# nikhilTkur/Multigrid_Nikhil_C-

Measured on AMD Instinct MI355X. Metric: fine_grid_stencil_updates_per_sec, higher is better.
Workload: dtype f64

## Files before the change

### multigrid_nikhil_c-_amd/csrc/mgx.hip

```cpp

#include "../../include/mgx.h"
#include "mgx_bottom.hpp"
#include "mgx_kernels.hpp"
#include "mgx_launch.hpp"
#include "mgx_var.hpp"
#include "mgx_galerkin.hpp"
#include "mgx_opdep.hpp"
#include "mgx_cheby.hpp"
#include "mgx_line.hpp"
#include "mgx_small.hpp"
#include "mgx_krylov.hpp"
#include "mgx_dist_plan.hpp"

#include <chrono>
#include <unistd.h>
#include <cmath>
#include <cstdio>
#include <cstdlib>
#include <cstring>
#include <string>
#include <vector>

namespace {

// ... 2018 lines not shown
    hipStream_t st = (hipStream_t)stream;
    int flips = 0;
    const int nb = with_kernel_set(q.f64, smoother, f->arith, [&](auto k) {
        using K = decltype(k);
        using T = typename K::T;
        return fold_block<T, K::SM, K::AR>(fc, q, (T*)u, (const T*)b, (T*)tmp, pitch, omega, c, (const T*)coarse_e,
                                           (T*)coarse_b, nullptr, crow_lo, crow_hi, restrict_mode, scratch, st, &flips);
    });
    if (nb < 0) return MGX_ERR_INVALID;
    if (post == 2) hipLaunchKernelGGL(k_reduce_partials, dim3(1), dim3(kReduceThreads), 0, st, scratch, nb, sum_dev);
    if (result_in_tmp) *result_in_tmp = flips & 1;
    return hipGetLastError() == hipSuccess ? MGX_OK : MGX_ERR_HIP;
}

int mgx_slab_restrict(const mgx_slab* f, const void* u, const void* b, const mgx_slab* c, void* cb, void* zero_u,
                      int crow_lo, int crow_hi, int restrict_mode, int fused, void* stream)
{
    if (slab_check(f) || slab_check(c) || !b || !cb || (fused && !u)) return MGX_ERR_INVALID;
    if (restrict_mode != MGX_RESTRICT_CONSISTENT && restrict_mode != MGX_RESTRICT_FW16) return MGX_ERR_INVALID;
    if (c->level != f->level - 1 || c->dtype != f->dtype) return MGX_ERR_INVALID;
    const int N = 1 << f->level;
    const long pitch = level_pitch(f->level, f->dtype), cpitch = level_pitch(c->level, c->dtype);
    const int off = 2 * c->row0 - f->row0;
    const int halo = fused ? 2 : 1;
    if (crow_lo < 0 || crow_hi > c->rows || crow_lo + c->row0 < 1 || crow_hi + c->row0 > N / 2) return MGX_ERR_INVALID;
    if (crow_hi > crow_lo && (2 * crow_lo + off - halo < 0 || 2 * (crow_hi - 1) + off + halo > f->rows - 1)) return MGX_ERR_INVALID;
    const int rpc = env_int("MGX_ROWS", 0);
    if (f->dtype == MGX_DTYPE_F64)
        launch_restrict<double>((const double*)u, (const double*)b, (double*)cb, (double*)zero_u, N, pitch, cpitch,
                                crow_lo, crow_hi, off, restrict_mode, fused != 0, rpc, (hipStream_t)stream);
    else
        launch_restrict<float>((const float*)u, (const float*)b, (float*)cb, (float*)zero_u, N, pitch, cpitch,
                               crow_lo, crow_hi, off, restrict_mode, fused != 0, rpc, (hipStream_t)stream);
    return hipGetLastError() == hipSuccess ? MGX_OK : MGX_ERR_HIP;
}

int mgx_slab_prolong(const mgx_slab* f, void* u, const mgx_slab* c, const void* e, int row_lo, int row_hi, int add,
                     void* stream)
{
    if (slab_check(f) || slab_check(c) || !u || !e) return MGX_ERR_INVALID;
    if (c->level != f->level - 1 || c->dtype != f->dtype) return MGX_ERR_INVALID;
    const int N = 1 << f->level;
    const long pitch = level_pitch(f->level, f->dtype), cpitch = level_pitch(c->level, c->dtype);
    const int off = 2 * c->row0 - f->row0;
    if (row_lo < 0 || row_hi > f->rows || row_lo + f->row0 < 1 || row_hi + f->row0 > N) return MGX_ERR_INVALID;
    if (row_hi > row_lo) {
        const int ylo = row_lo - off, yhi = row_hi - 1 - off;
        if (ylo < 0 || (yhi >> 1) + (yhi & 1) > c->rows - 1) return MGX_ERR_INVALID;
    }
    const int rpc = env_int("MGX_ROWS", 0);
    if (f->dtype == MGX_DTYPE_F64)
        launch_prolong<double>((double*)u, (const double*)e, N, pitch, cpitch, row_lo, row_hi, off, add != 0, rpc, (hipStream_t)stream);
    else
        launch_prolong<float>((float*)u, (const float*)e, N, pitch, cpitch, row_lo, row_hi, off, add != 0, rpc, (hipStream_t)stream);
    return hipGetLastError() == hipSuccess ? MGX_OK : MGX_ERR_HIP;
}

int mgx_slab_residual_sumsq(const mgx_slab* s, const void* u, const void* b, int row_lo, int row_hi,
                            double* scratch, double* sum_dev, void* stream)
{
    if (slab_check(s) || !u || !b || !scratch || !sum_dev) return MGX_ERR_INVALID;
    const int N = 1 << s->level;
    const long pitch = level_pitch(s->level, s->dtype);
    if (row_lo < 1 || row_hi > s->rows - 1 || row_lo + s->row0 < 1 || row_hi + s->row0 > N || row_hi <= row_lo) return MGX_ERR_INVALID;
    const int rpc = env_int("MGX_ROWS", 0);
    if (s->dtype == MGX_DTYPE_F64)
        launch_residual<double, 1>((const double*)u, (const double*)b, nullptr, 0, scratch, sum_dev, 1.0, N, pitch, row_lo, row_hi, rpc, (hipStream_t)stream, -1, s->rows);
    else
        launch_residual<float, 1>((const float*)u, (const float*)b, nullptr, 0, scratch, sum_dev, 1.0, N, pitch, row_lo, row_hi, rpc, (hipStream_t)stream, -1, s->rows);
    return hipGetLastError() == hipSuccess ? MGX_OK : MGX_ERR_HIP;
}

int mgx_create_rank(const mgx_config* cfg, int rank, int world, const void* rccl_id, const mgx_transport* transport,
                    mgx_handle* out)
{
    if (!cfg || !out) { g_create_error = "null argument"; return MGX_ERR_INVALID; }
    *out = nullptr;
    if (cfg->smoother == MGX_SMOOTHER_CHEBYSHEV) {
        g_create_error = "MGX_SMOOTHER_CHEBYSHEV: single-GPU handles of op = MGX_OPERATOR_STENCIL5 / MGX_OPERATOR_GALERKIN only";
        return MGX_ERR_INVALID;
    }
    if (cfg->smoother >= MGX_SMOOTHER_LINE_X && cfg->smoother <= MGX_SMOOTHER_LINE_ALT) {
        g_create_error = "MGX_SMOOTHER_LINE_X / LINE_Y / LINE_ALT: single-GPU handles of op = MGX_OPERATOR_STENCIL5 / MGX_OPERATOR_GALERKIN only";
        return MGX_ERR_INVALID;
    }
    if (cfg->coarsest_level < 2 || cfg->finest_level < cfg->coarsest_level || cfg->finest_level > 15 ||
        cfg->mu1 < 0 || cfg->mu2 < 0 || !(cfg->omega > 0.0 && cfg->omega < 2.0) || cfg->smoother < 0 || cfg->smoother > 1 ||
        cfg->dtype < 0 || cfg->dtype > 2 || cfg->restrict_mode < 0 || cfg->restrict_mode > 1 || cfg->bottom < 0 || cfg->bottom > 1 || cfg->arith < 0 || cfg->arith > 1 ||
        (rank >= 0 && (world < 1 || rank >= world)) || (rank < 0 && cfg->n_gpus < 2)) {
        g_create_error = "invalid configuration";
        return MGX_ERR_INVALID;
    }
    if (cfg->op != MGX_OPERATOR_POISSON) {
        g_create_error = "multi-GPU handles: op = MGX_OPERATOR_POISSON only (MGX_OPERATOR_STENCIL5 / MGX_OPERATOR_GALERKIN: one GPU)";
        return MGX_ERR_INVALID;
    }
    log_runtime_libs("mgx_create_rank");
    mgx_solver* s = new (std::nothrow) mgx_solver();
    if (!s) { g_create_error = "out of host memory"; return MGX_ERR_ALLOC; }
    s->cfg = *cfg;
    const int rc = dist_create(s, &s->cfg, rank, world, rccl_id, transport);
    if (rc != MGX_OK) { g_create_error = s->err; mgx_destroy(s); return rc; }
    *out = s;
    return MGX_OK;
}

int mgx_runtime_libs(char* buf, size_t cap)
{
    if (!buf || cap == 0) return -1;
    buf[0] = 0;
    FILE* fh = std::fopen("/proc/self/maps", "r");
    if (!fh) return -1;
    std::vector<std::string> seen;
    char line[4096];
    while (std::fgets(line, sizeof line, fh)) {
        const char* path = std::strchr(line, '/');
        if (!path) continue;
        std::string p(path);
        while (!p.empty() && (p.back() == '\n' || p.back() == ' ')) p.pop_back();
        const char* names[] = {"libamdhip64", "libhsa-runtime64", "librccl", "libmgx", "libhiprtc", "libamd_comgr"};
        bool want = false;
        for (const char* n : names) want = want || p.find(n) != std::string::npos;
        if (!want || std::find(seen.begin(), seen.end(), p) != seen.end()) continue;
        seen.push_back(p);
    }
    std::fclose(fh);
    std::string out;
    for (const auto& p : seen) { out += p; out += '\n'; }
    if (out.size() + 1 > cap) out.resize(cap - 1);
    std::memcpy(buf, out.c_str(), out.size() + 1);
    return (int)out.size();
}

int mgx_rccl_unique_id(void* out128)
{
    if (!out128) return MGX_ERR_INVALID;
    ncclUniqueId id;
    if (ncclGetUniqueId(&id) != ncclSuccess) return MGX_ERR_HIP;
    std::memset(out128, 0, 128);
    std::memcpy(out128, &id, sizeof(id) < 128 ? sizeof(id) : 128);
    return MGX_OK;
}

#ifdef MGX_WAVE_TRACE
__attribute__((visibility("default"))) int mgx_debug_wave_trace(void* out, int cap)
{
    int n = 0;
    if (hipDeviceSynchronize() != hipSuccess) return -1;
    if (hipMemcpyFromSymbol(&n, HIP_SYMBOL(mgx::g_wave_trace_n), sizeof(int)) != hipSuccess) return -1;
    n = std::min(std::min(n, cap), 1 << 16);
    if (hipMemcpyFromSymbol(out, HIP_SYMBOL(mgx::g_wave_trace), (size_t)n * sizeof(mgx::WaveTrace)) != hipSuccess) return -1;
    return n;
}
#endif

long mgx_dist_exchanges(mgx_handle s) { return (s && s->dist) ? s->dist->exchanges : -1; }
long mgx_dist_overlapped(mgx_handle s) { return (s && s->dist) ? s->dist->overlapped : -1; }

int mgx_memcpy_d2h(void* dst_host, const void* src_dev, size_t bytes, void* stream)
{
    if (hipMemcpyAsync(dst_host, src_dev, bytes, hipMemcpyDeviceToHost, (hipStream_t)stream) != hipSuccess) return MGX_ERR_HIP;
    return hipStreamSynchronize((hipStream_t)stream) == hipSuccess ? MGX_OK : MGX_ERR_HIP;
}

int mgx_memcpy_h2d(void* dst_dev, const void* src_host, size_t bytes, void* stream)
{
    if (hipMemcpyAsync(dst_dev, src_host, bytes, hipMemcpyHostToDevice, (hipStream_t)stream) != hipSuccess) return MGX_ERR_HIP;
    return hipStreamSynchronize((hipStream_t)stream) == hipSuccess ? MGX_OK : MGX_ERR_HIP;
}

struct mgx_dist_planner { mgx::DistPlanner p; };

int mgx_plan_create(const mgx_config* cfg, int n_slabs, int g, int fold, int deep, mgx_plan_handle* out)
{
    if (!cfg || !out) { g_plan_error = "null argument"; return MGX_ERR_INVALID; }
    *out = nullptr;
    if (cfg->smoother == MGX_SMOOTHER_CHEBYSHEV) {
        g_plan_error = "MGX_SMOOTHER_CHEBYSHEV: the slab plan runs the constant stencil (Jacobi or red-black GS) only";
        return MGX_ERR_INVALID;
    }
    if (cfg->smoother >= MGX_SMOOTHER_LINE_X && cfg->smoother <= MGX_SMOOTHER_LINE_ALT) {
        g_plan_error = "MGX_SMOOTHER_LINE_X / LINE_Y / LINE_ALT: the slab plan runs the constant stencil (Jacobi or red-black GS) only";
        return MGX_ERR_INVALID;
    }
    const int cut = dist_cut_level(*cfg, n_slabs);
    mgx_dist_planner* h = new (std::nothrow) mgx_dist_planner();
    if (!h) return MGX_ERR_ALLOC;
    if (h->p.init(plan_cfg_of(*cfg, n_slabs, g, cut, fold != 0, deep != 0)) != MGX_OK) {
        g_plan_error = h->p.err;
        delete h;
        return MGX_ERR_INVALID;
    }
    *out = h;
    return MGX_OK;
}

int mgx_plan_destroy(mgx_plan_handle p) { delete p; return MGX_OK; }
const char* mgx_plan_last_error(void) { return g_plan_error.c_str(); }
int mgx_plan_cut_level(mgx_plan_handle p) { return p ? p->p.c.cut : -1; }

int mgx_plan_level(mgx_plan_handle p, int level, mgx_dist_level* out)
{
    if (!p || !out || level <= p->p.c.cut || level > p->p.c.finest) return MGX_ERR_INVALID;
    *out = p->p.L(level);
    return MGX_OK;
}

int mgx_plan_cut_share(mgx_plan_handle p, int* row0, int* rows)
{
    if (!p || !row0 || !rows) return MGX_ERR_INVALID;
    *row0 = p->p.c_row0; *rows = p->p.c_rows;
    return MGX_OK;
}

int mgx_plan_guess_set(mgx_plan_handle p, int all_rows)
{
    if (!p) return MGX_ERR_INVALID;
    if (all_rows) p->p.guess_set(); else p->p.guess_changed();
    return MGX_OK;
}

static int plan_emit(mgx_plan_handle p, mgx_dist_op* ops, int cap, bool norm)
{
    if (!p || (!ops && cap > 0)) return MGX_ERR_INVALID;
    std::vector<mgx_dist_op> v;
    mgx::DistPlanner trial = p->p;
    if (norm) trial.emit_norm(v); else trial.emit_vcycle(v);
    if ((int)v.size() > cap) return -(int)v.size();
    p->p = trial;
    for (size_t i = 0; i < v.size(); ++i) ops[i] = v[i];
    return (int)v.size();
}
int mgx_plan_vcycle(mgx_plan_handle p, mgx_dist_op* ops, int cap) { return plan_emit(p, ops, cap, false); }
int mgx_plan_norm(mgx_plan_handle p, mgx_dist_op* ops, int cap) { return plan_emit(p, ops, cap, true); }
int mgx_plan_fmg(mgx_plan_handle p, mgx_dist_op* ops, int cap)
{
    if (!p || (!ops && cap > 0)) return MGX_ERR_INVALID;
    std::vector<mgx_dist_op> v;
    mgx::DistPlanner trial = p->p;
    trial.emit_fmg(v);
    if ((int)v.size() > cap) return -(int)v.size();
    p->p = trial;
    for (size_t i = 0; i < v.size(); ++i) ops[i] = v[i];
    return (int)v.size();
}

}
```

### multigrid_nikhil_c-_amd/csrc/mgx_bottom.hpp

```cpp
#pragma once

#include <hip/hip_runtime.h>
#include <cmath>
#include <vector>

#ifndef MGX_DST_DEEP
#define MGX_DST_DEEP 32
#endif

namespace mgx {

template <typename T, bool FIRST>
__global__ void __launch_bounds__(256)
k_dst_pair(const double* __restrict__ S, const void* __restrict__ Xv, void* __restrict__ Ov, const double* __restrict__ s,
           int n, long gpitch)
{
    __shared__ double prow[256];
    const int j = threadIdx.x;
    const int i = blockIdx.x;
    const bool live = j < n;
    constexpr int kDeep = MGX_DST_DEEP;
    const double* Sr = S + (long)i * n;
    double acc = 0.0;
    {
        int k = 0;
        for (; k + kDeep <= n; k += kDeep) {
            double x[kDeep];
#pragma unroll
            for (int q = 0; q < kDeep; ++q) {
                if constexpr (FIRST) x[q] = live ? (double)(reinterpret_cast<const T*>(Xv)[(long)(k + q + 1) * gpitch + (j + 1)]) : 0.0;
                else x[q] = live ? reinterpret_cast<const double*>(Xv)[(long)(k + q) * n + j] : 0.0;
            }
#pragma unroll
            for (int q = 0; q < kDeep; ++q) acc += Sr[k + q] * x[q];
        }
        double x[kDeep];
#pragma unroll
        for (int q = 0; q < kDeep; ++q) {
            const bool ok = live && (k + q < n);
            if constexpr (FIRST) x[q] = ok ? (double)(reinterpret_cast<const T*>(Xv)[(long)(k + q + 1) * gpitch + (j + 1)]) : 0.0;
            else x[q] = ok ? reinterpret_cast<const double*>(Xv)[(long)(k + q) * n + j] : 0.0;
        }
#pragma unroll
        for (int q = 0; q < kDeep; ++q)
            if (k + q < n) acc += Sr[k + q] * x[q];
    }
    prow[j] = acc;
    __syncthreads();
    double out = 0.0;
    {
        int k = 0;
        for (; k + kDeep <= n; k += kDeep) {
            double x[kDeep];
#pragma unroll
            for (int q = 0; q < kDeep; ++q) x[q] = live ? S[(long)(k + q) * n + j] : 0.0;
#pragma unroll
            for (int q = 0; q < kDeep; ++q) out += prow[k + q] * x[q];
        }
        double x[kDeep];
#pragma unroll
        for (int q = 0; q < kDeep; ++q) x[q] = (live && k + q < n) ? S[(long)(k + q) * n + j] : 0.0;
#pragma unroll
        for (int q = 0; q < kDeep; ++q)
            if (k + q < n) out += prow[k + q] * x[q];
    }
    if (!live) return;
    if constexpr (FIRST) reinterpret_cast<double*>(Ov)[(long)i * n + j] = out / (s[i] + s[j]);
    else reinterpret_cast<T*>(Ov)[(long)(i + 1) * gpitch + (j + 1)] = (T)out;
}

struct BottomDST {
    int n = 0;
    double* S = nullptr;
    double* s = nullptr;
    double* w1 = nullptr;

    hipError_t init(int n_)
    {
        n = n_;
        const size_t nn = (size_t)n * n;
        std::vector<double> hS(nn), hs(n);
        const long double pi = 3.14159265358979323846264338327950288L;
        const long double norm = sqrtl(2.0L / (long double)(n + 1));
        for (int i = 0; i < n; ++i) {
            const long double a = sinl(pi * (long double)(i + 1) / (2.0L * (long double)(n + 1)));
            hs[i] = (double)(4.0L * a * a);
            for (int k = 0; k < n; ++k) {
                const long m = ((long)(i + 1) * (long)(k + 1)) % (2L * (n + 1));
                hS[(size_t)i * n + k] = (double)(norm * sinl(pi * (long double)m / (long double)(n + 1)));
            }
        }
        hipError_t e;
        if ((e = hipMalloc(&S, nn * sizeof(double))) != hipSuccess) return e;
        if ((e = hipMalloc(&s, n * sizeof(double))) != hipSuccess) return e;
        if ((e = hipMalloc(&w1, nn * sizeof(double))) != hipSuccess) return e;
        if ((e = hipMemcpy(S, hS.data(), nn * sizeof(double), hipMemcpyHostToDevice)) != hipSuccess) return e;
        if ((e = hipMemcpy(s, hs.data(), n * sizeof(double), hipMemcpyHostToDevice)) != hipSuccess) return e;
        return hipSuccess;
    }

    void destroy()
    {
        if (S) (void)hipFree(S);
        if (s) (void)hipFree(s);
        if (w1) (void)hipFree(w1);
        S = s = w1 = nullptr;
    }

    template <typename T>
    void solve(const T* b_grid, T* u_grid, long gpitch, hipStream_t st) const
    {
        hipLaunchKernelGGL((k_dst_pair<T, true>), dim3(n), dim3(256), 0, st, S, (const void*)b_grid, (void*)w1, s, n, gpitch);
        hipLaunchKernelGGL((k_dst_pair<T, false>), dim3(n), dim3(256), 0, st, S, (const void*)w1, (void*)u_grid, s, n, gpitch);
    }
};

}
```

### multigrid_nikhil_c-_amd/csrc/mgx_kernels.hpp

```cpp
#pragma once

#include <hip/hip_runtime.h>
#include "mgx_geom.hpp"
#include <stdint.h>
#include <type_traits>

namespace mgx {

template <int B, int E, typename F> __device__ __forceinline__ void static_for(F&& f)
{
    if constexpr (B < E) {
        f(std::integral_constant<int, B>{});
        static_for<B + 1, E>(f);
    }
}

constexpr int kWave = 64;
constexpr int kBlock = 256;
constexpr int kWavesPerBlock = kBlock / kWave;
constexpr int kOutLanes = kWave - 2;

template <typename T> struct VecOf;
template <> struct VecOf<double> { using type = double2; static constexpr int W = 2; };
template <> struct VecOf<float>  { using type = float4;  static constexpr int W = 4; };

__device__ __forceinline__ double2 vzero(double2*) { return make_double2(0.0, 0.0); }
__device__ __forceinline__ float4  vzero(float4*)  { return make_float4(0.f, 0.f, 0.f, 0.f); }

template <typename V> __device__ __forceinline__ V vload(const void* p, bool pred)
{
    V z = vzero((V*)nullptr);
    if (pred) z = *reinterpret_cast<const V*>(p);
    return z;
}
template <typename V> __device__ __forceinline__ void vstore(void* p, const V& v, bool pred)
{
    if (pred) *reinterpret_cast<V*>(p) = v;
}

__device__ __forceinline__ double first(const double2& v) { return v.x; }
__device__ __forceinline__ double last(const double2& v)  { return v.y; }
__device__ __forceinline__ float  first(const float4& v)  { return v.x; }
__device__ __forceinline__ float  last(const float4& v)   { return v.w; }

__device__ __forceinline__ int dpp_shr1(int x) { return __builtin_amdgcn_update_dpp(0, x, 0x138, 0xf, 0xf, true); }
__device__ __forceinline__ int dpp_shl1(int x) { return __builtin_amdgcn_update_dpp(0, x, 0x130, 0xf, 0xf, true); }
__device__ __forceinline__ float from_left(float x)  { return __int_as_float(dpp_shr1(__float_as_int(x))); }
__device__ __forceinline__ float from_right(float x) { return __int_as_float(dpp_shl1(__float_as_int(x))); }
__device__ __forceinline__ double from_left(double x)
{
    return __hiloint2double(dpp_shr1(__double2hiint(x)), dpp_shr1(__double2loint(x)));
}
__device__ __forceinline__ double from_right(double x)
{
    return __hiloint2double(dpp_shl1(__double2hiint(x)), dpp_shl1(__double2loint(x)));
}

#ifndef MGX_SOFF_LOADS
#define MGX_SOFF_LOADS 1
#endif
typedef int v4i32 __attribute__((ext_vector_type(4)));
typedef int v2i32 __attribute__((ext_vector_type(2)));
constexpr unsigned kOobOffset = 0xFFFFFF00u;
__device__ __forceinline__ __amdgpu_buffer_rsrc_t make_rsrc(const void* p, unsigned bytes)
{
    return __builtin_amdgcn_make_buffer_rsrc(const_cast<void*>(p), 0, (int)bytes, 0x00020000);
}
__device__ __forceinline__ void bstore(const double2& v, __amdgpu_buffer_rsrc_t r, unsigned voff)
{
    const v4i32 t = {__double2loint(v.x), __double2hiint(v.x), __double2loint(v.y), __double2hiint(v.y)};
    __builtin_amdgcn_raw_buffer_store_b128(t, r, voff, 0, 0);
}
__device__ __forceinline__ void bstore(const float4& v, __amdgpu_buffer_rsrc_t r, unsigned voff)
{
    const v4i32 t = {__float_as_int(v.x), __float_as_int(v.y), __float_as_int(v.z), __float_as_int(v.w)};
    __builtin_amdgcn_raw_buffer_store_b128(t, r, voff, 0, 0);
}
__device__ __forceinline__ void bstore8(double v, __amdgpu_buffer_rsrc_t r, unsigned voff)
{
    const v2i32 t = {__double2loint(v), __double2hiint(v)};
    __builtin_amdgcn_raw_buffer_store_b64(t, r, voff, 0, 0);
}
__device__ __forceinline__ void bstore8(float2 v, __amdgpu_buffer_rsrc_t r, unsigned voff)
{
    const v2i32 t = {__float_as_int(v.x), __float_as_int(v.y)};
    __builtin_amdgcn_raw_buffer_store_b64(t, r, voff, 0, 0);
}
__device__ __forceinline__ double2 bload(double2*, __amdgpu_buffer_rsrc_t r, unsigned voff)
{
    const v4i32 t = __builtin_amdgcn_raw_buffer_load_b128(r, voff, 0, 0);
    return make_double2(__hiloint2double(t.y, t.x), __hiloint2double(t.w, t.z));
}
__device__ __forceinline__ float4 bload(float4*, __amdgpu_buffer_rsrc_t r, unsigned voff)
{
    const v4i32 t = __builtin_amdgcn_raw_buffer_load_b128(r, voff, 0, 0);
    return make_float4(__int_as_float(t.x), __int_as_float(t.y), __int_as_float(t.z), __int_as_float(t.w));
}
__device__ __forceinline__ double2 bload_s(double2*, __amdgpu_buffer_rsrc_t r, unsigned voff, unsigned soff)
{
    const v4i32 t = __builtin_amdgcn_raw_buffer_load_b128(r, voff, soff, 0);
    return make_double2(__hiloint2double(t.y, t.x), __hiloint2double(t.w, t.z));
}
__device__ __forceinline__ float4 bload_s(float4*, __amdgpu_buffer_rsrc_t r, unsigned voff, unsigned soff)
{
    const v4i32 t = __builtin_amdgcn_raw_buffer_load_b128(r, voff, soff, 0);
    return make_float4(__int_as_float(t.x), __int_as_float(t.y), __int_as_float(t.z), __int_as_float(t.w));
}
__device__ __forceinline__ double bload1_s(double*, __amdgpu_buffer_rsrc_t r, unsigned voff, unsigned soff)
{
    const v2i32 t = __builtin_amdgcn_raw_buffer_load_b64(r, voff, soff, 0);
    return __hiloint2double(t.y, t.x);
}
__device__ __forceinline__ float bload1_s(float*, __amdgpu_buffer_rsrc_t r, unsigned voff, unsigned soff)
{
    return __int_as_float(__builtin_amdgcn_raw_buffer_load_b32(r, voff, soff, 0));
}
__device__ __forceinline__ double bload1(double*, __amdgpu_buffer_rsrc_t r, unsigned voff)
{
    const v2i32 t = __builtin_amdgcn_raw_buffer_load_b64(r, voff, 0, 0);
    return __hiloint2double(t.y, t.x);
}
__device__ __forceinline__ float bload1(float*, __amdgpu_buffer_rsrc_t r, unsigned voff)
{
    return __int_as_float(__builtin_amdgcn_raw_buffer_load_b32(r, voff, 0, 0));
}

struct FastOut {
    __amdgpu_buffer_rsrc_t out, cb, cz;
    __amdgpu_buffer_rsrc_t in, rhs, ce;
    unsigned lane_off;
    unsigned clane_off;
    unsigned pitch_bytes, cpitch_bytes;
    int rb, crb;
};
__device__ __forceinline__ unsigned rsrc_bytes(int first, int last, unsigned long row_bytes)
{
    if (last < first) return 0u;
    const unsigned long b = (unsigned long)(last - first + 1) * row_bytes;
    return b < 0x7FFFFF00ul ? (unsigned)b : 0x7FFFFF00u;
}
__device__ __forceinline__ int opaque_s(int x) { asm volatile("" : "+s"(x)); return x; }
struct ColMask { bool first, all; };
__device__ __forceinline__ ColMask col_mask(long col, int N) { return ColMask{col == 0, col >= N}; }
__device__ __forceinline__ void mask_sel(double2& v, const ColMask& m, bool row_zero)
{
    v.x = (m.first || m.all || row_zero) ? 0.0 : v.x;
    v.y = (m.all || row_zero) ? 0.0 : v.y;
}
__device__ __forceinline__ void mask_sel(float4& v, const ColMask& m, bool row_zero)
{
    v.x = (m.first || m.all || row_zero) ? 0.f : v.x;
    v.y = (m.all || row_zero) ? 0.f : v.y;
    v.z = (m.all || row_zero) ? 0.f : v.z;
    v.w = (m.all || row_zero) ? 0.f : v.w;
}

// ... 1296 lines not shown
    const int wv = __builtin_amdgcn_readfirstlane(threadIdx.x >> 6);
    const int ty = blockIdx.x / tiles_x, tx = blockIdx.x - ty * tiles_x;
    const int y0 = wv * RW;
    const int gy0 = row_lo + ty * TH - He + y0;
    const int gx = 1 + tx * TW - He + lane;
    const bool colunk = gx > 0 && gx < N;
    const int NC = N / 2;

    T u[RW], b[RW];
    unsigned rowmask = 0;
#pragma unroll
    for (int i = 0; i < RW; ++i) {
        const int gy = gy0 + i;
        const bool rowok = gy > 0 && gy < N && gy >= win.row_first && gy <= win.row_last;
        if (rowok) rowmask |= 1u << i;
        const bool unk = colunk && rowok;
        const long at = (long)gy * pitch + gx;
        u[i] = (unk && !zero_in) ? vin[at] : (T)0;
        b[i] = unk ? rhs[at] : (T)0;
    }
    if (PRE) {
        const bool codd = (gx & 1) != 0;
#pragma unroll
        for (int i = 0; i < RW; ++i) {
            const int gy = gy0 + i;
            const bool rodd = (gy & 1) != 0;
            const bool unk = colunk && ((rowmask >> i) & 1u) && (gy >> 1) >= win.crow_first && (gy >> 1) + (rodd ? 1 : 0) <= win.crow_last;
            const T* e = coarse_e + (long)(gy >> 1) * cpitch + (gx >> 1);
            const T a00 = unk ? e[0] : (T)0;
            const T a01 = (unk && codd) ? e[1] : (T)0;
            const T a10 = (unk && rodd) ? e[cpitch] : (T)0;
            const T a11 = (unk && rodd && codd) ? e[cpitch + 1] : (T)0;
            const T ev = codd ? (T)0.5 * (a00 + a01) : a00;
            const T od = codd ? (T)0.25 * (((a00 + a10) + a01) + a11) : (T)0.5 * (a00 + a10);
            const T add = rodd ? od : ev;
            u[i] = unk ? u[i] + add : u[i];
        }
    }

    int buf = 0;
    auto halo_rows = [&](const T (&a)[RW], T& up, T& dn) {
        edge[buf][wv][0][lane] = a[0];
        edge[buf][wv][1][lane] = a[RW - 1];
        __syncthreads();
        up = wv > 0 ? edge[buf][wv - 1][1][lane] : (T)0;
        dn = wv < kWavesPerBlock - 1 ? edge[buf][wv + 1][0][lane] : (T)0;
        buf ^= 1;
    };
    for (int j = 1; j <= levels; ++j) {
        T up, dn;
        halo_rows(u, up, dn);
        const bool colact = colunk && lane >= j && lane < kTileSX - j;
        const int ilo = max(j - y0, 0), ihi = min(kTileSY - j - y0, RW);
        const unsigned act = ihi > ilo ? (rowmask & (((1u << (ihi - ilo)) - 1u) << ilo)) : 0u;
        T prev = up;
#pragma unroll
        for (int i = 0; i < RW; ++i) {
            const T cur = u[i];
            const T below = (i == RW - 1) ? dn : u[i + 1];
            const T l = from_left(cur), r = from_right(cur);
            const bool rowact = (act >> i) & 1u;
            if (SM == 0) {
                const T o = jac_pt<AR>(c0, cur, c1 * b[i], c1, nbr(prev, l, r, below));
                u[i] = (colact && rowact) ? o : cur;
            } else {
                const T o = (T)0.25 * (b[i] + nbr(prev, l, r, below));
                u[i] = (colact && rowact && ((gy0 + i + gx) & 1) == ((j - 1) & 1)) ? o : cur;
            }
            prev = cur;
        }
    }

    const bool colout = lane >= He && lane < He + TW && gx < N;
#pragma unroll
    for (int i = 0; i < RW; ++i) {
        const int y = y0 + i, gy = gy0 + i;
        if (y >= He && y < He + TH && gy < N && gy >= row_lo && gy < row_hi && colout) vout[(long)gy * pitch + gx] = u[i];
    }

    if (POST != 0) {
        T up, dn;
        halo_rows(u, up, dn);
        T res[RW];
        double acc = 0.0;
        T prev = up;
#pragma unroll
        for (int i = 0; i < RW; ++i) {
            const T cur = u[i];
            const T below = (i == RW - 1) ? dn : u[i + 1];
            const int y = y0 + i, gy = gy0 + i;
            const T l = from_left(cur), r = from_right(cur);
            T rr = (T)0;
            if (colunk && gy > 0 && gy < N) rr = b[i] - (-nbr(prev, l, r, below) + (T)4 * cur);
            res[i] = rr;
            if (POST == 2 && y >= He && y < He + TH && gy >= row_lo && gy < row_hi && colout) acc += (double)rr * (double)rr;
            prev = cur;
        }
        if (POST == 2) {
            for (int off = 32; off > 0; off >>= 1) acc += __shfl_down(acc, off, kWave);
            if (lane == 0) wsum[wv] = acc;
            __syncthreads();
            if (threadIdx.x == 0) {
                double sum = 0.0;
                for (int w2 = 0; w2 < kWavesPerBlock; ++w2) sum += wsum[w2];
                partial[blockIdx.x] = sum;
            }
        }
        if (POST == 1) {
            T rup, rdn;
            halo_rows(res, rup, rdn);
            const int J = gx >> 1;
            const bool cst = colout && (gx & 1) == 0 && J >= 1 && J < NC;
#pragma unroll
            for (int i = 0; i < RW; ++i) {
                const T c = res[i];
                const T n = (i == 0) ? rup : res[i - 1];
                const T s2 = (i == RW - 1) ? rdn : res[i + 1];
                const int y = y0 + i, gy = gy0 + i;
                T corners = from_left(n) + from_right(n);
                corners = corners + from_left(s2);
                corners = corners + from_right(s2);
                T edges = from_left(c) + from_right(c);
                edges = edges + n;
                edges = edges + s2;
                const T o = wgt * ((corners + (T)2 * edges) + (T)4 * c);
                if (cst && y >= He && y < He + TH && (gy & 1) == 0 && gy < N && gy >= row_lo && gy < row_hi &&
                    (gy >> 1) >= win.emit_lo && (gy >> 1) < win.emit_hi) {
                    const long at = (long)(gy >> 1) * cpitch + J;
                    coarse_b[at] = o;
                    if (coarse_zero) coarse_zero[at] = (T)0;
                }
            }
        }
    }
}

__device__ __forceinline__ double vget(const double2& v, int e) { return e == 0 ? v.x : v.y; }
__device__ __forceinline__ float vget(const float4& v, int e) { return e == 0 ? v.x : (e == 1 ? v.y : (e == 2 ? v.z : v.w)); }
__device__ __forceinline__ double2 vmake(const double (&a)[2]) { return make_double2(a[0], a[1]); }
__device__ __forceinline__ float4 vmake(const float (&a)[4]) { return make_float4(a[0], a[1], a[2], a[3]); }

template <typename T, int SM, int PRE, int POST, int AR, int RW>
__global__ void __launch_bounds__(kTileWideWaves * kWave)
k_tile_wide(const T* __restrict__ vin, const T* __restrict__ rhs, T* __restrict__ vout,
            const T* __restrict__ coarse_e, T* __restrict__ coarse_b, T* __restrict__ coarse_zero, T wgt,
            double* __restrict__ partial, int N, long pitch, long cpitch, int levels, T c0, T c1,
            int tiles_x, int zero_in, int row_lo, int row_hi, CycleWin win)
{
    using V = typename VecOf<T>::type;
    constexpr int W = VecOf<T>::W;
    constexpr int NW = kTileWideWaves;
    __shared__ V edge[2][NW][2][kWave];
    __shared__ double wsum[NW];
    const TileWideGeom g = tile_wide_geom(N, row_lo, row_hi, levels + tile_extra<POST>(), W, RW);
    const int He = g.He, TH = g.TH, TW = g.TW;
    const int lane = threadIdx.x & 63;
    const int wv = __builtin_amdgcn_readfirstlane(threadIdx.x >> 6);
    const int ty = blockIdx.x / tiles_x, tx = blockIdx.x - ty * tiles_x;
    const int y0 = wv * RW;
    const int gy0 = row_lo + ty * TH - He + y0;
    const int cx0 = tx * TW;
    const int gx0 = cx0 - g.Hx + W * lane;
    const bool vld = gx0 >= 0 && gx0 < N;
    const bool cu0 = vld && gx0 > 0;
    bool cu[W];
#pragma unroll
    for (int e = 0; e < W; ++e) cu[e] = e == 0 ? cu0 : vld;
    const int NC = N / 2;

    T u[RW][W], b[RW][W];
    unsigned rowmask = 0;
#pragma unroll
    for (int i = 0; i < RW; ++i) {
        const int gy = gy0 + i;
        const bool rowok = gy > 0 && gy < N && gy >= win.row_first && gy <= win.row_last;
        if (rowok) rowmask |= 1u << i;
        const long at = (long)gy * pitch + gx0;
        V uv = vzero((V*)nullptr), bv = vzero((V*)nullptr);
        if (vld && rowok) {
            bv = *reinterpret_cast<const V*>(rhs + at);
            if (!zero_in) uv = *reinterpret_cast<const V*>(vin + at);
        }
#pragma unroll
        for (int e = 0; e < W; ++e) {
            u[i][e] = cu[e] ? vget(uv, e) : (T)0;
            b[i][e] = cu[e] ? vget(bv, e) : (T)0;
        }
    }
    if (PRE) {
        constexpr int NCR = RW / 2 + 1, NCC = W / 2 + 1;
        const int kc0 = gy0 >> 1, J = gx0 >> 1;
        T cr[NCR][NCC];
#pragma unroll
        for (int k = 0; k < NCR; ++k) {
            const int cy = kc0 + k;
            const bool ok = vld && cy >= 0 && cy <= NC && cy >= win.crow_first && cy <= win.crow_last;
            const T* ep = coarse_e + (long)cy * cpitch + J;
#pragma unroll
            for (int m = 0; m < NCC; ++m) cr[k][m] = ok ? ep[m] : (T)0;
        }
        auto correct = [&](auto parity) {
            constexpr int par = decltype(parity)::value;
#pragma unroll
            for (int i = 0; i < RW; ++i) {
                const int gy = gy0 + i;
                const bool rodd = ((par + i) & 1) != 0;
                const int kr = (par + i) >> 1;
                const bool rin = ((rowmask >> i) & 1u) && (gy >> 1) >= win.crow_first && (gy >> 1) + (rodd ? 1 : 0) <= win.crow_last;
#pragma unroll
                for (int e = 0; e < W; ++e) {
                    const bool codd = (e & 1) != 0;
                    const bool unk = cu[e] && rin;
                    const T a00 = unk ? cr[kr][e >> 1] : (T)0;
                    const T a01 = (unk && codd) ? cr[kr][(e >> 1) + 1] : (T)0;
                    const T a10 = (unk && rodd) ? cr[kr + (rodd ? 1 : 0)][e >> 1] : (T)0;
                    const T a11 = (unk && rodd && codd) ? cr[kr + (rodd ? 1 : 0)][(e >> 1) + 1] : (T)0;
                    const T ev = codd ? (T)0.5 * (a00 + a01) : a00;
                    const T od = codd ? (T)0.25 * (((a00 + a10) + a01) + a11) : (T)0.5 * (a00 + a10);
                    const T add = rodd ? od : ev;
                    u[i][e] = unk ? u[i][e] + add : u[i][e];
                }
            }
        };
        if (gy0 & 1) correct(std::integral_constant<int, 1>{});
        else correct(std::integral_constant<int, 0>{});
    }

    int buf = 0;
    auto halo_rows = [&](const T (&a)[RW][W], T (&up)[W], T (&dn)[W]) {
        edge[buf][wv][0][lane] = vmake(a[0]);
        edge[buf][wv][1][lane] = vmake(a[RW - 1]);
        __syncthreads();
        const V uv = wv > 0 ? edge[buf][wv - 1][1][lane] : vzero((V*)nullptr);
        const V dv = wv < NW - 1 ? edge[buf][wv + 1][0][lane] : vzero((V*)nullptr);
#pragma unroll
        for (int e = 0; e < W; ++e) { up[e] = vget(uv, e); dn[e] = vget(dv, e); }
        buf ^= 1;
    };
    for (int j = 1; j <= levels; ++j) {
        T up[W], dn[W];
        halo_rows(u, up, dn);
        const int colour = (j - 1) & 1;
        T prev[W];
#pragma unroll
        for (int e = 0; e < W; ++e) prev[e] = up[e];
#pragma unroll
        for (int i = 0; i < RW; ++i) {
            T cur[W];
#pragma unroll
            for (int e = 0; e < W; ++e) cur[e] = u[i][e];
            const T l = from_left(cur[W - 1]), r = from_right(cur[0]);
            const bool rowact = (rowmask >> i) & 1u;
#pragma unroll
            for (int e = 0; e < W; ++e) {
                const T below = (i == RW - 1) ? dn[e] : u[i + 1][e];
                const T we = e == 0 ? l : cur[e - 1], ea = e == W - 1 ? r : cur[e + 1];
                if (SM == 0) {
                    const T o = jac_pt<AR>(c0, cur[e], c1 * b[i][e], c1, nbr(prev[e], we, ea, below));
                    u[i][e] = (cu[e] && rowact) ? o : cur[e];
                } else {
                    const T o = (T)0.25 * (b[i][e] + nbr(prev[e], we, ea, below));
                    u[i][e] = (cu[e] && rowact && ((gy0 + i + e) & 1) == colour) ? o : cur[e];
                }
            }
#pragma unroll
            for (int e = 0; e < W; ++e) prev[e] = cur[e];
        }
    }

    const bool colout = gx0 >= cx0 && gx0 < cx0 + TW && gx0 < N;
#pragma unroll
    for (int i = 0; i < RW; ++i) {
        const int y = y0 + i, gy = gy0 + i;
        if (y >= He && y < He + TH && gy < N && gy >= row_lo && gy < row_hi && colout)
            *reinterpret_cast<V*>(vout + (long)gy * pitch + gx0) = vmake(u[i]);
    }

    if (POST != 0) {
        T up[W], dn[W];
        halo_rows(u, up, dn);
        T res[RW][W];
        double acc = 0.0;
        T prev[W];
#pragma unroll
        for (int e = 0; e < W; ++e) prev[e] = up[e];
#pragma unroll
        for (int i = 0; i < RW; ++i) {
            const int y = y0 + i, gy = gy0 + i;
            const T l = from_left(u[i][W - 1]), r = from_right(u[i][0]);
            const bool rowunk = gy > 0 && gy < N;
            const bool rowout = POST == 2 && y >= He && y < He + TH && gy >= row_lo && gy < row_hi && colout;
#pragma unroll
            for (int e = 0; e < W; ++e) {
                const T cur = u[i][e];
                const T below = (i == RW - 1) ? dn[e] : u[i + 1][e];
                const T we = e == 0 ? l : u[i][e - 1], ea = e == W - 1 ? r : u[i][e + 1];
                T rr = (T)0;
                if (cu[e] && rowunk) rr = b[i][e] - (-nbr(prev[e], we, ea, below) + (T)4 * cur);
                res[i][e] = rr;
                if (rowout) acc += (double)rr * (double)rr;
            }
#pragma unroll
            for (int e = 0; e < W; ++e) prev[e] = u[i][e];
        }
        if (POST == 2) {
            for (int off = 32; off > 0; off >>= 1) acc += __shfl_down(acc, off, kWave);
            if (lane == 0) wsum[wv] = acc;
            __syncthreads();
            if (threadIdx.x == 0) {
                double sum = 0.0;
                for (int w2 = 0; w2 < NW; ++w2) sum += wsum[w2];
                partial[blockIdx.x] = sum;
            }
        }
        if (POST == 1) {
            T rup[W], rdn[W];
            halo_rows(res, rup, rdn);
#pragma unroll
            for (int i = 0; i < RW; ++i) {
                const int y = y0 + i, gy = gy0 + i;
                const bool rowst = y >= He && y < He + TH && (gy & 1) == 0 && gy < N && gy >= row_lo && gy < row_hi &&
                                   (gy >> 1) >= win.emit_lo && (gy >> 1) < win.emit_hi;
                T n[W], s2[W];
#pragma unroll
                for (int e = 0; e < W; ++e) {
                    n[e] = (i == 0) ? rup[e] : res[i - 1][e];
                    s2[e] = (i == RW - 1) ? rdn[e] : res[i + 1][e];
                }
                const T nl = from_left(n[W - 1]), sl = from_left(s2[W - 1]), cl = from_left(res[i][W - 1]);
#pragma unroll
                for (int e = 0; e < W; e += 2) {
                    const T c = res[i][e];
                    T corners = (e == 0 ? nl : n[e - 1]) + n[e + 1];
                    corners = corners + (e == 0 ? sl : s2[e - 1]);
                    corners = corners + s2[e + 1];
                    T edges = (e == 0 ? cl : res[i][e - 1]) + res[i][e + 1];
                    edges = edges + n[e];
                    edges = edges + s2[e];
                    const T o = wgt * ((corners + (T)2 * edges) + (T)4 * c);
                    const int J = (gx0 + e) >> 1;
                    if (rowst && colout && J >= 1 && J < NC) {
                        const long at = (long)(gy >> 1) * cpitch + J;
                        coarse_b[at] = o;
                        if (coarse_zero) coarse_zero[at] = (T)0;
                    }
                }
            }
        }
    }
}

static __global__ void __launch_bounds__(kBlock)
k_axpy_f32_to_f64(double* __restrict__ u, const float* __restrict__ e, double scale, int N, long pitch, long epitch,
                  int row_lo, int row_hi, int R, int strips, int chunks, int assign)
{
    const Tile t = wave_tile(strips, chunks);
    if (!t.active) return;
    const Cols c = lane_cols<2>(t.strip, N, pitch);
    const int r0 = row_lo + t.chunk * R;
    const int r1 = min(r0 + R, row_hi);
    for (int r = r0; r < r1; ++r) {
        if (c.st) {
            const float2 ev = *reinterpret_cast<const float2*>(e + (long)r * epitch + c.col);
            double2* pu = reinterpret_cast<double2*>(u + (long)r * pitch + c.col);
            double2 o = assign ? make_double2(0.0, 0.0) : *pu;
            o.x = o.x + scale * (double)ev.x;
            o.y = o.y + scale * (double)ev.y;
            if (c.col == 0) o.x = 0.0;
            *pu = o;
        }
    }
}

static __global__ void __launch_bounds__(kBlock)
k_update_residual(const double* __restrict__ u, const float* __restrict__ e, const double* __restrict__ rhs,
                  double* __restrict__ unew, float* __restrict__ r32, double scale, double inv_scale,
                  double* __restrict__ partial, int N, long pitch, long epitch, int row_lo, int row_hi,
                  int R, int strips, int chunks)
{
    __shared__ double wsum[kWavesPerBlock];
    const Tile t = wave_tile(strips, chunks);
    double acc = 0.0;
    if (t.active) {
        const Cols c = lane_cols<2>(t.strip, N, pitch);
        const int r0 = row_lo + t.chunk * R;
        const int r1 = min(r0 + R, row_hi);
        auto updated = [&](int r) {
            double2 o = make_double2(0.0, 0.0);
            if (c.ld) {
                const double2 uv = *reinterpret_cast<const double2*>(u + (long)r * pitch + c.col);
                const float2 ev = *reinterpret_cast<const float2*>(e + (long)r * epitch + c.col);
                o.x = uv.x + scale * (double)ev.x;
                o.y = uv.y + scale * (double)ev.y;
                if (c.col == 0) o.x = 0.0;
            }
            return o;
        };
        double2 up = updated(r0 - 1);
        double2 cur = updated(r0);
        for (int r = r0; r < r1; ++r) {
            const double2 dn = updated(r + 1);
            const double2 bb = vload<double2>(rhs + (long)r * pitch + c.col, c.ld);
            double2 o = residual_vec(up, cur, dn, bb);
            mask_cols(o, c.col, N);
            if (c.st) {
                *reinterpret_cast<double2*>(unew + (long)r * pitch + c.col) = cur;
                acc += (double)o.x * (double)o.x + (double)o.y * (double)o.y;
                *reinterpret_cast<float2*>(r32 + (long)r * epitch + c.col) =
                    make_float2((float)(o.x * inv_scale), (float)(o.y * inv_scale));
            }
            up = cur; cur = dn;
        }
    }
    for (int off = 32; off > 0; off >>= 1) acc += __shfl_down(acc, off, kWave);
    if ((threadIdx.x & 63) == 0) wsum[threadIdx.x >> 6] = acc;
    __syncthreads();
    if (threadIdx.x == 0) {
        double s = 0.0;
        for (int w = 0; w < kWavesPerBlock; ++w) s += wsum[w];
        partial[blockIdx.x] = s;
    }
}

static __global__ void __launch_bounds__(kBlock)
k_scale_f64_to_f32(float* __restrict__ out, const double* __restrict__ in, double inv_scale, int N, long pitch_in, long pitch_out,
                   int row_lo, int row_hi, int R, int strips, int chunks)
{
    const Tile t = wave_tile(strips, chunks);
    if (!t.active) return;
    const Cols c = lane_cols<2>(t.strip, N, pitch_in);
    const int r0 = row_lo + t.chunk * R;
    const int r1 = min(r0 + R, row_hi);
    for (int r = r0; r < r1; ++r) {
        if (c.st) {
            double2 x = *reinterpret_cast<const double2*>(in + (long)r * pitch_in + c.col);
            if (c.col == 0) x.x = 0.0;
            *reinterpret_cast<float2*>(out + (long)r * pitch_out + c.col) =
                make_float2((float)(x.x * inv_scale), (float)(x.y * inv_scale));
        }
    }
}

struct Launch { int R, strips, chunks, blocks; };

inline Launch make_launch(int N, int W, int rows, int rows_per_chunk)
{
    Launch L;
    const int nvec_out = N / W;
    L.strips = (nvec_out + kOutLanes - 1) / kOutLanes;
    if (L.strips < 1) L.strips = 1;
    int R = rows_per_chunk;
    if (R <= 0) {
        R = rows / 128;
        if (R < 4) R = 4;
        if (R > 8) R = 8;
    }
    L.R = R;
    L.chunks = (rows + R - 1) / R;
    if (L.chunks < 1) L.chunks = 1;
    const long waves = (long)L.strips * L.chunks;
    long blocks = (waves + kWavesPerBlock - 1) / kWavesPerBlock;
    blocks = (blocks + 7) / 8 * 8;
    L.blocks = (int)blocks;
    return L;
}

}
```

Baseline: 1109 billion.

## Rework DST bottom solve with buffer loads, double-buffered prefetch and phase tracing

Rewrites the bottom-level DST pair kernel to use raw buffer loads with clamped offsets in place of predicated global loads. The matrix-vector dot product is double-buffered so the next batch of column loads is issued before the current batch is accumulated, and the second pass's first batch of S is prefetched during the first pass. The S row is staged in shared memory and the block size is sized to n instead of a fixed 256. It also adds compile-time-gated phase-timing instrumentation to the DST and tile kernels, which compiles to nothing by default. The costs are higher register pressure from two in-flight load batches and reliance on buffer-resource out-of-bounds semantics for inactive lanes.

```diff
diff --git a/multigrid_nikhil_c-_amd/csrc/mgx.hip b/multigrid_nikhil_c-_amd/csrc/mgx.hip
--- a/multigrid_nikhil_c-_amd/csrc/mgx.hip
+++ b/multigrid_nikhil_c-_amd/csrc/mgx.hip
@@ -2194,6 +2194,18 @@
     if (hipMemcpyFromSymbol(out, HIP_SYMBOL(mgx::g_wave_trace), (size_t)n * sizeof(mgx::WaveTrace)) != hipSuccess) return -1;
     return n;
 }
+__attribute__((visibility("default"))) int mgx_debug_phase_trace(void* out, int cap)
+{
+    unsigned n = 0;
+    if (hipDeviceSynchronize() != hipSuccess) return -1;
+    if (hipMemcpyFromSymbol(&n, HIP_SYMBOL(mgx::g_phase_trace_n), sizeof(n)) != hipSuccess) return -1;
+    std::vector<mgx::PhaseTrace> ring(mgx::kPhaseCap);
+    if (hipMemcpyFromSymbol(ring.data(), HIP_SYMBOL(mgx::g_phase_trace), ring.size() * sizeof(mgx::PhaseTrace)) != hipSuccess) return -1;
+    const unsigned have = std::min<unsigned>(n, mgx::kPhaseCap), take = std::min<unsigned>(have, (unsigned)std::max(cap, 0));
+    for (unsigned q = 0; q < take; ++q)
+        static_cast<mgx::PhaseTrace*>(out)[q] = ring[(n - take + q) & (mgx::kPhaseCap - 1)];
+    return (int)take;
+}
 #endif
 
 long mgx_dist_exchanges(mgx_handle s) { return (s && s->dist) ? s->dist->exchanges : -1; }
diff --git a/multigrid_nikhil_c-_amd/csrc/mgx_bottom.hpp b/multigrid_nikhil_c-_amd/csrc/mgx_bottom.hpp
--- a/multigrid_nikhil_c-_amd/csrc/mgx_bottom.hpp
+++ b/multigrid_nikhil_c-_amd/csrc/mgx_bottom.hpp
@@ -2,7 +2,10 @@
 
 #include <hip/hip_runtime.h>
 #include <cmath>
+#include <type_traits>
 #include <vector>
+
+#include "mgx_phase_trace.hpp"
 
 #ifndef MGX_DST_DEEP
 #define MGX_DST_DEEP 32
@@ -10,63 +13,108 @@
 
 namespace mgx {
 
+constexpr unsigned kDstOob = 0xFFFFFF00u;
+__device__ __forceinline__ __amdgpu_buffer_rsrc_t dst_rsrc(const void* p, unsigned bytes)
+{
+    return __builtin_amdgcn_make_buffer_rsrc(const_cast<void*>(p), 0, (int)bytes, 0x00020000);
+}
+template <typename E> __device__ __forceinline__ double dst_load(__amdgpu_buffer_rsrc_t r, unsigned voff, unsigned soff)
+{
+    if constexpr (sizeof(E) == 8) {
+        const auto t = __builtin_amdgcn_raw_buffer_load_b64(r, voff, soff, 0);
+        return __hiloint2double(t[1], t[0]);
+    } else {
+        return (double)__int_as_float(__builtin_amdgcn_raw_buffer_load_b32(r, voff, soff, 0));
+    }
+}
+template <typename E, int D>
+__device__ __forceinline__ void dst_batch(double (&x)[D], __amdgpu_buffer_rsrc_t r, unsigned voff, unsigned rowbytes, int k0, int n)
+{
+    const unsigned last = (unsigned)(n - 1) * rowbytes;
+    unsigned off = (unsigned)k0 * rowbytes;
+#pragma unroll
+    for (int q = 0; q < D; ++q, off += rowbytes) x[q] = dst_load<E>(r, voff, min(off, last));
+}
+template <int CNT, int D> __device__ __forceinline__ void dst_chain(double& acc, const double* m, const double (&x)[D])
+{
+#pragma unroll
+    for (int q = 0; q < CNT; ++q) acc += m[q] * x[q];
+}
+template <int D> __device__ __forceinline__ void dst_chain_last(double& acc, const double* m, const double (&x)[D], int rem)
+{
+    if (rem == D - 1) {
+        dst_chain<D - 1>(acc, m, x);
+    } else {
+#pragma unroll
+        for (int q = 0; q < D; ++q)
+            if (q < rem) acc += m[q] * x[q];
+    }
+}
+template <int D, typename Load, typename Before, typename Stamp>
+__device__ __forceinline__ double dst_dot(const double* m, int n, double (&xa)[D], Load load, Before before_last, Stamp landed)
+{
+    double xb[D];
+    double acc = 0.0;
+    int k = 0;
+    for (;;) {
+        if (k + D >= n) { before_last(); landed(xa[D - 1]); dst_chain_last<D>(acc, m + k, xa, n - k); break; }
+        load(xb, k + D);
+        landed(xa[D - 1]);
+        dst_chain<D, D>(acc, m + k, xa);
+        k += D;
+        if (k + D >= n) { before_last(); landed(xb[D - 1]); dst_chain_last<D>(acc, m + k, xb, n - k); break; }
+        load(xa, k + D);
+        landed(xb[D - 1]);
+        dst_chain<D, D>(acc, m + k, xb);
+        k += D;
+    }
+    return acc;
+}
+
 template <typename T, bool FIRST>
 __global__ void __launch_bounds__(256)
 k_dst_pair(const double* __restrict__ S, const void* __restrict__ Xv, void* __restrict__ Ov, const double* __restrict__ s,
            int n, long gpitch)
 {
-    __shared__ double prow[256];
+    using E = std::conditional_t<FIRST, T, double>;
+    __shared__ double srow[256], prow[256];
+    MGX_PHASE_BEGIN();
     const int j = threadIdx.x;
     const int i = blockIdx.x;
     const bool live = j < n;
     constexpr int kDeep = MGX_DST_DEEP;
-    const double* Sr = S + (long)i * n;
-    double acc = 0.0;
-    {
-        int k = 0;
-        for (; k + kDeep <= n; k += kDeep) {
-            double x[kDeep];
-#pragma unroll
-            for (int q = 0; q < kDeep; ++q) {
-                if constexpr (FIRST) x[q] = live ? (double)(reinterpret_cast<const T*>(Xv)[(long)(k + q + 1) * gpitch + (j + 1)]) : 0.0;
-                else x[q] = live ? reinterpret_cast<const double*>(Xv)[(long)(k + q) * n + j] : 0.0;
-            }
-#pragma unroll
-            for (int q = 0; q < kDeep; ++q) acc += Sr[k + q] * x[q];
-        }
-        double x[kDeep];
-#pragma unroll
-        for (int q = 0; q < kDeep; ++q) {
-            const bool ok = live && (k + q < n);
-            if constexpr (FIRST) x[q] = ok ? (double)(reinterpret_cast<const T*>(Xv)[(long)(k + q + 1) * gpitch + (j + 1)]) : 0.0;
-            else x[q] = ok ? reinterpret_cast<const double*>(Xv)[(long)(k + q) * n + j] : 0.0;
-        }
-#pragma unroll
-        for (int q = 0; q < kDeep; ++q)
-            if (k + q < n) acc += Sr[k + q] * x[q];
+    const unsigned srb = (unsigned)n * 8u, xrb = FIRST ? (unsigned)gpitch * (unsigned)sizeof(T) : srb;
+    const char* xp = static_cast<const char*>(Xv) + (FIRST ? (gpitch + 1) * (long)sizeof(T) : 0L);
+    const __amdgpu_buffer_rsrc_t rs = dst_rsrc(S, (unsigned)n * srb);
+    const __amdgpu_buffer_rsrc_t rx = dst_rsrc(xp, (unsigned)(n - 1) * xrb + (unsigned)n * (unsigned)sizeof(E));
+    const unsigned vs = live ? (unsigned)j * 8u : kDstOob, vx = live ? (unsigned)j * (unsigned)sizeof(E) : kDstOob;
+    auto landed = [&](const double& v) { MGX_PHASE_AFTER(v); (void)v; };
+
+    const double si = dst_load<double>(rs, vs, (unsigned)i * srb);
+    double ei = 0.0, ej = 0.0;
+    if constexpr (FIRST) {
+        const __amdgpu_buffer_rsrc_t re = dst_rsrc(s, srb);
+        ei = dst_load<double>(re, live ? 0u : kDstOob, (unsigned)i * 8u);
+        ej = dst_load<double>(re, vs, 0u);
     }
+    double xa[kDeep], s2[kDeep];
+    dst_batch<E, kDeep>(xa, rx, vx, xrb, 0, n);
+    srow[j] = si;
+    __syncthreads();
+    const double acc = dst_dot<kDeep>(srow, n, xa, [&](double (&x)[kDeep], int k0) { dst_batch<E, kDeep>(x, rx, vx, xrb, k0, n); },
+                                      [&]() { dst_batch<double, kDeep>(s2, rs, vs, srb, 0, n); }, landed);
+    MGX_PHASE_AFTER(acc);
     prow[j] = acc;
     __syncthreads();
-    double out = 0.0;
-    {
-        int k = 0;
-        for (; k + kDeep <= n; k += kDeep) {
-            double x[kDeep];
-#pragma unroll
-            for (int q = 0; q < kDeep; ++q) x[q] = live ? S[(long)(k + q) * n + j] : 0.0;
-#pragma unroll
-            for (int q = 0; q < kDeep; ++q) out += prow[k + q] * x[q];
-        }
-        double x[kDeep];
-#pragma unroll
-        for (int q = 0; q < kDeep; ++q) x[q] = (live && k + q < n) ? S[(long)(k + q) * n + j] : 0.0;
-#pragma unroll
-        for (int q = 0; q < kDeep; ++q)
-            if (k + q < n) out += prow[k + q] * x[q];
+    MGX_PHASE();
+    const double out = dst_dot<kDeep>(prow, n, s2, [&](double (&x)[kDeep], int k0) { dst_batch<double, kDeep>(x, rs, vs, srb, k0, n); },
+                                      []() {}, landed);
+    MGX_PHASE_AFTER(out);
+    if (live) {
+        if constexpr (FIRST) reinterpret_cast<double*>(Ov)[(long)i * n + j] = out / (ei + ej);
+        else reinterpret_cast<T*>(Ov)[(long)(i + 1) * gpitch + (j + 1)] = (T)out;
     }
-    if (!live) return;
-    if constexpr (FIRST) reinterpret_cast<double*>(Ov)[(long)i * n + j] = out / (s[i] + s[j]);
-    else reinterpret_cast<T*>(Ov)[(long)(i + 1) * gpitch + (j + 1)] = (T)out;
+    MGX_PHASE_END(kPhaseDst, n | (FIRST ? 1 << 16 : 0));
 }
 
 struct BottomDST {
@@ -110,8 +158,9 @@
     template <typename T>
     void solve(const T* b_grid, T* u_grid, long gpitch, hipStream_t st) const
     {
-        hipLaunchKernelGGL((k_dst_pair<T, true>), dim3(n), dim3(256), 0, st, S, (const void*)b_grid, (void*)w1, s, n, gpitch);
-        hipLaunchKernelGGL((k_dst_pair<T, false>), dim3(n), dim3(256), 0, st, S, (const void*)w1, (void*)u_grid, s, n, gpitch);
+        const int block = (n + 63) / 64 * 64;
+        hipLaunchKernelGGL((k_dst_pair<T, true>), dim3(n), dim3(block), 0, st, S, (const void*)b_grid, (void*)w1, s, n, gpitch);
+        hipLaunchKernelGGL((k_dst_pair<T, false>), dim3(n), dim3(block), 0, st, S, (const void*)w1, (void*)u_grid, s, n, gpitch);
     }
 };
 
diff --git a/multigrid_nikhil_c-_amd/csrc/mgx_kernels.hpp b/multigrid_nikhil_c-_amd/csrc/mgx_kernels.hpp
--- a/multigrid_nikhil_c-_amd/csrc/mgx_kernels.hpp
+++ b/multigrid_nikhil_c-_amd/csrc/mgx_kernels.hpp
@@ -2,6 +2,7 @@
 
 #include <hip/hip_runtime.h>
 #include "mgx_geom.hpp"
+#include "mgx_phase_trace.hpp"
 #include <stdint.h>
 #include <type_traits>
 
@@ -1604,6 +1605,7 @@
     constexpr int NW = kTileWideWaves;
     __shared__ V edge[2][NW][2][kWave];
     __shared__ double wsum[NW];
+    MGX_PHASE_BEGIN();
     const TileWideGeom g = tile_wide_geom(N, row_lo, row_hi, levels + tile_extra<POST>(), W, RW);
     const int He = g.He, TH = g.TH, TW = g.TW;
     const int lane = threadIdx.x & 63;
@@ -1619,6 +1621,7 @@
 #pragma unroll
     for (int e = 0; e < W; ++e) cu[e] = e == 0 ? cu0 : vld;
     const int NC = N / 2;
+    MGX_PHASE_AFTER(gx0 + gy0);
 
     T u[RW][W], b[RW][W];
     unsigned rowmask = 0;
@@ -1678,6 +1681,9 @@
         else correct(std::integral_constant<int, 0>{});
     }
 
+    MGX_PHASE_AFTER(b[RW - 1][W - 1]);
+    MGX_PHASE_AFTER(u[RW - 1][W - 1]);
+
     int buf = 0;
     auto halo_rows = [&](const T (&a)[RW][W], T (&up)[W], T (&dn)[W]) {
         edge[buf][wv][0][lane] = vmake(a[0]);
@@ -1718,6 +1724,7 @@
 #pragma unroll
             for (int e = 0; e < W; ++e) prev[e] = cur[e];
         }
+        MGX_PHASE_AFTER(u[RW - 1][W - 1]);
     }
 
     const bool colout = gx0 >= cx0 && gx0 < cx0 + TW && gx0 < N;
@@ -1727,6 +1734,7 @@
         if (y >= He && y < He + TH && gy < N && gy >= row_lo && gy < row_hi && colout)
             *reinterpret_cast<V*>(vout + (long)gy * pitch + gx0) = vmake(u[i]);
     }
+    MGX_PHASE();
 
     if (POST != 0) {
         T up[W], dn[W];
@@ -1755,6 +1763,7 @@
 #pragma unroll
             for (int e = 0; e < W; ++e) prev[e] = u[i][e];
         }
+        MGX_PHASE_AFTER(res[RW - 1][W - 1]);
         if (POST == 2) {
             for (int off = 32; off > 0; off >>= 1) acc += __shfl_down(acc, off, kWave);
             if (lane == 0) wsum[wv] = acc;
@@ -1800,6 +1809,7 @@
             }
         }
     }
+    MGX_PHASE_END(kPhaseTile, N | (PRE << 16) | (POST << 20) | (RW << 24));
 }
 
 static __global__ void __launch_bounds__(kBlock)
diff --git a/multigrid_nikhil_c-_amd/csrc/mgx_phase_trace.hpp b/multigrid_nikhil_c-_amd/csrc/mgx_phase_trace.hpp
--- /dev/null
+++ b/multigrid_nikhil_c-_amd/csrc/mgx_phase_trace.hpp
@@ -0,0 +1,47 @@
+#pragma once
+
+#include <hip/hip_runtime.h>
+
+#ifdef MGX_WAVE_TRACE
+namespace mgx {
+
+constexpr int kPhaseMax = 24;
+constexpr int kPhaseCap = 1 << 14;
+constexpr int kPhaseDst = 0, kPhaseTile = 1;
+struct PhaseTrace { int kind, tag, block, n; long long t[kPhaseMax]; };
+__device__ PhaseTrace g_phase_trace[kPhaseCap];
+__device__ unsigned g_phase_trace_n;
+
+__device__ __forceinline__ void phase_mark(long long* t, int& n)
+{
+    if (threadIdx.x < 64) {
+        const long long c = wall_clock64();
+        if (threadIdx.x == 0 && n < kPhaseMax) t[n] = c;
+    }
+    ++n;
+}
+template <typename X> __device__ __forceinline__ void phase_mark_after(long long* t, int& n, const X& v)
+{
+    asm volatile("" ::"v"(v) : "memory");
+    phase_mark(t, n);
+}
+__device__ __forceinline__ void phase_flush(const long long* t, int n, int kind, int tag)
+{
+    if (threadIdx.x == 0) {
+        PhaseTrace& r = g_phase_trace[atomicAdd(&g_phase_trace_n, 1u) & (kPhaseCap - 1)];
+        r.kind = kind; r.tag = tag; r.block = (int)blockIdx.x; r.n = n < kPhaseMax ? n : kPhaseMax;
+        for (int q = 0; q < r.n; ++q) r.t[q] = t[q];
+    }
+}
+
+}
+#define MGX_PHASE_BEGIN() __shared__ long long ph_t[mgx::kPhaseMax]; int ph_n = 0; mgx::phase_mark(ph_t, ph_n)
+#define MGX_PHASE() mgx::phase_mark(ph_t, ph_n)
+#define MGX_PHASE_AFTER(v) mgx::phase_mark_after(ph_t, ph_n, (v))
+#define MGX_PHASE_END(kind, tag) (mgx::phase_mark(ph_t, ph_n), mgx::phase_flush(ph_t, ph_n, (kind), (tag)))
+#else
+#define MGX_PHASE_BEGIN() ((void)0)
+#define MGX_PHASE() ((void)0)
+#define MGX_PHASE_AFTER(v) ((void)0)
+#define MGX_PHASE_END(kind, tag) ((void)0)
+#endif
```

Result: faster. 1122 billion, median of 6 (+1.1%).
